# tammypi/flink-siddhi

Measured on AMD Instinct MI355X. Metric: matched-pattern events/sec (whole node) at 1/2/4/8 MI355X + % HBM roofline, higher is better.
Workload: dtype f64+int32+int64

## Files before the change

flink-siddhi_amd/csrc/cf_kernels.hip:

```cpp
#include <hip/hip_runtime.h>

#include "dev_common.h"
#include "kernels.h"
#include "vm.h"

namespace cep {

namespace {

constexpr uint16_t kNoB = 0xffff;
constexpr uint32_t kRolePB = 4;
constexpr int64_t kTolBias = 1ll << 31;
constexpr uint32_t kSkrAlive = 0x8000u;
constexpr int kCfStageBytes = (kCfTile / 8192 * 20 + 36) * 1024;

#ifdef CF_WAVESTAMP
#define CF_STAMP(i) do { } while (0)
#else
#define CF_STAMP(i)                                                                 \
  do {                                                                              \
    if (a.stamps && threadIdx.x == 0 && blockIdx.x < 4096)                          \
      a.stamps[(int64_t)blockIdx.x * 16 + (i)] = __builtin_amdgcn_s_memtime();      \
  } while (0)
#endif

#ifdef CF_WAVESTAMP
#define CF_WSTAMP(slot)                                                             \
  do {                                                                              \
    if (a.stamps && (threadIdx.x & 63) == 0 && blockIdx.x < 4096 && wi == 0 &&     \
        (slot) < 16)                                                                \
      a.stamps[(int64_t)blockIdx.x * 16 + (slot)] = __builtin_amdgcn_s_memtime();  \
  } while (0)
#else
#define CF_WSTAMP(slot) do { } while (0)
#endif

#define CF_COUNT(i, v)                                                                       \
  do {                                                                                       \
    if (a.stamps && (a.ablate & 256))                                                        \
      atomicAdd((unsigned long long*)&a.stamps[4095 * 16 + (i)], (unsigned long long)(v));   \
  } while (0)

template <int E, int Q = kPref>
__device__ __forceinline__ void pick_carried(const uint64_t (&pv)[Q][E], int sa, int sb,
                                             uint32_t role_a, uint64_t (&out)[E]) {
  take_slot<E, Q>(pv, sa, out);
  if (sb != sa) {
#pragma unroll
    for (int q = 0; q < Q; ++q) {
      if (sb == q) {
        asm volatile("");
#pragma unroll
        for (int e = 0; e < E; ++e) out[e] = ((role_a >> e) & 1u) ? out[e] : pv[q][e];
      }
    }
  }
}

__device__ __forceinline__ uint32_t rec_row(uint64_t w0) { return (uint32_t)(w0 >> 32) & 0x1fffu; }
__device__ __forceinline__ uint32_t rec_role(uint64_t w0) { return (uint32_t)(w0 >> 45) & 0x7u; }
__device__ __forceinline__ uint32_t rec_key(uint64_t w0) { return (uint32_t)(w0 >> 48); }

}

#ifndef CF_PART_MINW
#define CF_PART_MINW (kCfPartThreads == 512 ? 4 : 1)
#endif
template <int NW, bool FR, int NP = kPref, bool TOL = false, bool ATL = false>
__global__ __launch_bounds__(kCfPartThreads, CF_PART_MINW) void k_cfpart(CfPartArgs a) {
  constexpr int E = kCfItems, NT = kCfPartThreads, RW = 1 + NW;
  constexpr int kStageBytesT = (FR || TOL || ATL) ? 128 * 1024 : kCfStageBytes;
  constexpr int kStageRecs = kStageBytesT / (8 * RW);
  constexpr uint64_t kHwmBias = 1ull << 63;
  __shared__ uint32_t scratch[NT / 64 + 1];
  __shared__ unsigned long long s_hwm;
  __shared__ unsigned long long s_wmax[NT / 64];
  __shared__ __attribute__((aligned(16))) uint64_t stage[kStageRecs * RW];
  extern __shared__ __attribute__((aligned(16))) uint32_t hist[];
  const int tid = threadIdx.x;
  const int64_t tile = xcd_tile(blockIdx.x, a.ntiles);
  if (TOL && a.gate && *(volatile const uint32_t*)a.gate != a.gate_seq) return;
  const PatternArgs& p = a.pat;
  const bool need_hwm = (ATL && (tile == 0 || tile == a.ntiles - 1)) || (TOL && a.hwm_wr);
  if (need_hwm) {
    if (tid < 64) {
      unsigned long long h = a.hwm_rd ? a.hwm_rd[tid] : 0ull;
#pragma unroll
      for (int o = 32; o > 0; o >>= 1) {
        const unsigned long long y = __shfl_xor(h, o, 64);
        h = y > h ? y : h;
      }
      if (tid == 0) s_hwm = h;
    }
    __syncthreads();
  }
  const int lg = p.buckets_log2;
  const int P = 1 << lg;
  const int NB = P + a.nhot;
  CF_STAMP(0);
  for (int i = tid; i <= NB; i += NT) hist[i] = 0;

  const int64_t ts_base = FR ? (int64_t)a.in_recs[a.rows.row0 * a.in_rec_words + 2] : a.rows.ts[a.rows.row0];
  if (tile == 0 && tid == 0) {
    if (a.pool_cursor) *a.pool_cursor = 0ull;
    a.chunk_base[0] = ts_base;
    a.chunk_base[1] = FR ? (int64_t)a.in_recs[a.rows.row0 * a.in_rec_words + 1] : a.rows.seq0 + a.rows.row0;
  }
  const int lane = tid & 63, wave = tid >> 6;
  const int64_t r0 = tile * kCfTile + (int64_t)wave * 64 * E + lane;
  const int64_t row0 = a.rows.row0 + r0;
  uint32_t valid = 0;
#pragma unroll
  for (int e = 0; e < E; ++e) valid |= (r0 + 64 * e < a.rows.n ? 1u : 0u) << e;
  uint32_t role_a = 0, role_b = 0, role_pb = 0;
  uint64_t tsv[E];
  uint64_t pv[NP][E];
#pragma unroll
  for (int e = 0; e < E; ++e) tsv[e] = 0;
  uint64_t fkey[E], fc0[E], fc1[E];
#pragma unroll
  for (int e = 0; e < E; ++e) fkey[e] = fc0[e] = fc1[e] = 0;
  if (FR && valid) {
    const int rw = a.in_rec_words;
    uint64_t hv[E];
#pragma unroll
    for (int e = 0; e < E; ++e) {
      const bool ok = (valid >> e) & 1u;
      const uint64_t* r = a.in_recs + (row0 + 64 * e) * rw;
      hv[e] = ok ? r[0] : 0ull;
      tsv[e] = ok ? r[2] : 0ull;
      const bool isa = ((hv[e] >> 32) & ROLE_A) != 0;
      fc0[e] = (ok && NW > 0) ? r[3 + (isa ? a.cf.a_log[0] : a.cf.b_log[0])] : 0ull;
      fc1[e] = (ok && NW > 1) ? r[3 + (isa ? a.cf.a_log[1] : a.cf.b_log[1])] : 0ull;
    }
#pragma unroll
    for (int e = 0; e < E; ++e) {
      const uint32_t role = (uint32_t)(hv[e] >> 32) & 0xffu;
      role_a |= ((role & ROLE_A) ? 1u : 0u) << e;
      role_b |= ((role & ROLE_B) && (role & ROLE_G) ? 1u : 0u) << e;
      if (TOL) role_pb |= ((role & ROLE_B) && !(role & ROLE_G) ? 1u : 0u) << e;
      fkey[e] = (uint64_t)(uint32_t)hv[e];
    }
    if (p.within >= 0 && !TOL) {
      const int64_t before = row0 > 0 ? (int64_t)a.in_recs[(row0 - 1) * rw + 2] : batch_prev_ts(a.rows);
      bool bad = false;
#pragma unroll
      for (int e = 0; e < E; ++e) {
        const uint64_t up = __shfl_up(tsv[e], 1, 64);
        const uint64_t last = e > 0 ? __shfl(tsv[e > 0 ? e - 1 : 0], 63, 64) : 0ull;
        const int64_t prev = lane > 0 ? (int64_t)up : (e > 0 ? (int64_t)last : before);
        if ((valid >> e) & 1u) bad |= (int64_t)tsv[e] < prev;
      }
      if (bad) report_descent(a.rows, a.err);
    }
  }
  if (!FR && valid) {
    uint32_t sb[E];
    cf_load_cols<E, NP>(a.rows, a.pref, a.ts_slot, row0, valid, tsv, sb, pv);
    uint32_t is_a = 0, is_b = 0;
#pragma unroll
    for (int e = 0; e < E; ++e) {
      if ((valid >> e) & 1u) {
        is_a |= ((int)sb[e] == p.a_stream ? 1u : 0u) << e;
        is_b |= ((int)sb[e] == p.b_stream ? 1u : 0u) << e;
      }
    }
    if (p.within >= 0 && !TOL) {
      int64_t before;
      if (ATL && r0 == 0) {
        before = (int64_t)(s_hwm ^ kHwmBias);
      } else {
        before = row0 > 0 ? a.rows.ts[row0 - 1] : batch_prev_ts(a.rows);
      }
      bool bad = false;
#pragma unroll
      for (int e = 0; e < E; ++e) {
        const uint64_t up = __shfl_up(tsv[e], 1, 64);
        const uint64_t last = e > 0 ? __shfl(tsv[e > 0 ? e - 1 : 0], 63, 64) : 0ull;
        const int64_t prev = lane > 0 ? (int64_t)up : (e > 0 ? (int64_t)last : before);
        if ((valid >> e) & 1u) bad |= (int64_t)tsv[e] < prev;
      }
      if (bad) {
        if (ATL) *(volatile uint32_t*)a.gate = a.gate_seq;
        else report_descent(a.rows, a.err);
      }
    }
    const uint32_t all = (1u << E) - 1u;
    if (is_a) role_a = is_a & (p.f_prog < 0 ? all : eval_terms_regs<E, NP>(p.f_terms, a.pref.f_slot, a.rows.cols, pv));
    if (is_b) role_b = is_b & (p.g_raw_prog < 0 ? all : eval_terms_regs<E, NP>(p.g_terms, a.pref.g_slot, a.rows.cols, pv));
    if (TOL || ATL) role_pb = is_b & ~role_b;
    if (NW > 0) pick_carried<E, NP>(pv, a.cf.a_slot[0], a.cf.b_slot[0], role_a, fc0);
    if (NW > 1) pick_carried<E, NP>(pv, a.cf.a_slot[1], a.cf.b_slot[1], role_a, fc1);
    if (a.pref.key_slot >= 0) {
#pragma unroll
      for (int e = 0; e < E; ++e) fkey[e] = pv[0][e];
    }
  }
  if (TOL && a.hwm_wr) {
    unsigned long long m = 0ull;
#pragma unroll
    for (int e = 0; e < E; ++e)
      if ((valid >> e) & 1u) m = (tsv[e] ^ kHwmBias) > m ? (tsv[e] ^ kHwmBias) : m;
#pragma unroll
    for (int o = 32; o > 0; o >>= 1) {
      const unsigned long long y = __shfl_xor(m, o, 64);
      m = y > m ? y : m;
    }
    if (lane == 0) s_wmax[wave] = m;
  }
  lds_barrier();
  CF_STAMP(1);
  if (TOL && a.hwm_wr && tid == 0) {
    unsigned long long m = s_hwm;
    for (int w = 0; w < NT / 64; ++w) m = s_wmax[w] > m ? s_wmax[w] : m;
    atomicMax(a.hwm_wr + (tile & 63), m);
  }
  if (ATL && tile == a.ntiles - 1 && tid == 0) {
    const unsigned long long l = (unsigned long long)a.rows.ts[a.rows.row0 + a.rows.n - 1] ^ kHwmBias;
    a.hwm_wr[0] = l > s_hwm ? l : s_hwm;
  }

  uint32_t packed[E];
  uint32_t lkey[E];
#pragma unroll
  for (int e = 0; e < E; ++e) {
    packed[e] = 0xffffffffu;
    lkey[e] = 0;
    const uint32_t role = ((role_a >> e) & 1u) * ROLE_A | ((role_b >> e) & 1u) * ROLE_B |
                          ((TOL || ATL) ? ((role_pb >> e) & 1u) * kRolePB : 0u);
    if (!role) continue;
    int64_t key;
    key = (int64_t)fkey[e];
    const int64_t kfield = shard_key(key, p.key_stride, p.key_offset);
    if (kfield < 0 || kfield >= p.key_capacity) {
      set_err(a.err, ERR_KEY_RANGE);
      continue;
    }
    uint32_t bucket = (uint32_t)(kfield & (P - 1));
    lkey[e] = (uint32_t)(kfield >> lg);
    if (ATL) {
      if (role == kRolePB) bucket += (uint32_t)P;
    } else if (a.nhot) {
      const uint32_t hs = a.hot_id[kfield];
      if (hs != kNotHot) {
        bucket = (uint32_t)P + hs;
        lkey[e] = hs;
      }
    }
    const uint32_t rank = atomicAdd(&hist[bucket], 1u);
    packed[e] = (role << 25) | (bucket << 13) | rank;
  }
  lds_barrier();
  CF_STAMP(2);
  {
    constexpr int MAXPER = kCfMaxBuckets / NT;
    const int per = (NB + NT - 1) / NT;
    uint32_t c[MAXPER];
    uint32_t sum = 0;
#pragma unroll
    for (int i = 0; i < MAXPER; ++i) {
      const int idx = tid * per + i;
      c[i] = (i < per && idx < NB) ? hist[idx] : 0u;
      sum += c[i];
    }
    uint32_t total;
    uint32_t off = bscan<NT>(sum, scratch, &total);
#pragma unroll
    for (int i = 0; i < MAXPER; ++i) {
      const int idx = tid * per + i;
      if (i < per && idx < NB) {
        hist[idx] = off;
        off += c[i];
      }
    }
    if (tid == 0) hist[NB] = total;
  }
  lds_barrier();
  CF_STAMP(3);
  const uint32_t total = hist[NB];
  const uint32_t nreg = ATL ? hist[P] : total;
  const uint32_t words_t = nreg * RW + (total - nreg);
  const bool staged = words_t <= (uint32_t)(kStageRecs * RW);
  uint64_t* trecs = a.recs + tile * (int64_t)kCfTile * RW;
#pragma unroll
  for (int e = 0; e < E; ++e) {
    if (packed[e] == 0xffffffffu) continue;
    const uint32_t b = (packed[e] >> 13) & 0xfffu;
    const uint32_t role = packed[e] >> 25;
    const uint32_t slot = hist[b] + (packed[e] & 0x1fffu);
    const int64_t dts = (int64_t)tsv[e] - ts_base + (TOL ? kTolBias : 0);
    if (dts < 0) {
      if (TOL) set_err(a.err, ERR_TS_SPAN);
      else if (ATL) *(volatile uint32_t*)a.gate = a.gate_seq;
      else report_descent(a.rows, a.err);
    } else if (dts > 0xffffffffll) {
      set_err(a.err, ERR_TS_SPAN);
    }
    const uint64_t w0 = (uint64_t)(uint32_t)dts | ((uint64_t)(wave * 64 * E + 64 * e + lane) << 32) |
                        ((uint64_t)role << 45) | ((uint64_t)lkey[e] << 48);
    const uint64_t c0 = fc0[e], c1 = fc1[e];
    if (ATL && b >= (uint32_t)P) {
      const uint32_t wd = nreg * RW + (slot - nreg);
      if (staged) stage[wd] = w0;
      else trecs[wd] = w0;
      continue;
    }
    if (staged) {
      stage[slot * RW] = w0;
      if (NW > 0) stage[slot * RW + 1] = c0;
      if (NW > 1) stage[slot * RW + 2] = c1;
    } else {
      uint64_t* g = trecs + (int64_t)slot * RW;
      g[0] = w0;
      if (NW > 0) g[1] = c0;
      if (NW > 1) g[2] = c1;
    }
  }
  for (int i = tid; i <= NB; i += NT) a.tile_off[(int64_t)i * a.ntiles + tile] = (uint16_t)hist[i];
  if (staged) {
    lds_barrier();
    CF_STAMP(4);
    const int64_t words = (int64_t)words_t;
    for (int64_t w = 2 * tid; w < words; w += 2 * NT) {
      if (w + 1 < words) *(uint4*)(trecs + w) = *(const uint4*)(stage + w);
      else trecs[w] = stage[w];
    }
  }
  CF_STAMP(5);
}

#if !defined(CF_UNIT) || CF_UNIT == 1
constexpr int kCfRouteStage = 112 * 1024;
constexpr int kRouteSmallWorld = 8;
__global__ __launch_bounds__(kCfPartThreads, 1) void k_cfroute(CfRouteArgs ca) {
  constexpr int E = kCfItems, NT = kCfPartThreads, NWV = NT / 64;
  const RouteArgs& a = ca.r;
  const PatternArgs& p = a.pat;
  __shared__ uint32_t wcnt[NWV][kMaxWorld];
  __shared__ uint32_t obase[kMaxWorld + 1];
  __shared__ __attribute__((aligned(16))) uint64_t stage[kCfRouteStage / 8];
  const int tid = threadIdx.x, lane = tid & 63, wave = tid >> 6;
  const int world = a.world, wrw = a.wrw;
  const int64_t tile = blockIdx.x;
  for (int i = tid; i < NWV * kMaxWorld; i += NT) wcnt[i / kMaxWorld][i % kMaxWorld] = 0;

  const int64_t r0 = tile * kCfTile + (int64_t)wave * 64 * E + lane;
  const int64_t row0 = a.rows.row0 + r0;
  uint32_t valid = 0;
#pragma unroll
  for (int e = 0; e < E; ++e) valid |= (r0 + 64 * e < a.rows.n ? 1u : 0u) << e;
  uint64_t tsv[E], pv[kPref][E];
#pragma unroll
  for (int e = 0; e < E; ++e) tsv[e] = 0;
  uint32_t is_a = 0, role_a = 0, role_b = 0, role_g = 0;
  uint64_t fkey[E], fc0[E], fc1[E];
#pragma unroll
  for (int e = 0; e < E; ++e) fkey[e] = fc0[e] = fc1[e] = 0;
  if (valid) {
    uint32_t sb[E];
    cf_load_cols<E>(a.rows, ca.pref, ca.ts_slot, row0, valid, tsv, sb, pv);
    uint32_t is_b = 0;
#pragma unroll
    for (int e = 0; e < E; ++e) {
      if ((valid >> e) & 1u) {
        is_a |= ((int)sb[e] == p.a_stream ? 1u : 0u) << e;
        is_b |= ((int)sb[e] == p.b_stream ? 1u : 0u) << e;
      }
    }
    const uint32_t all = (1u << E) - 1u;
    if (is_a) role_a = is_a & (p.f_prog < 0 ? all : eval_terms_regs<E>(p.f_terms, ca.pref.f_slot, a.rows.cols, pv));
    if (is_b) {
      if (p.g_walk_prog >= 0) {
        role_b = is_b;
      } else {
        role_g = is_b & (p.g_raw_prog < 0 ? all : eval_terms_regs<E>(p.g_terms, ca.pref.g_slot, a.rows.cols, pv));
        role_b = p.tolerant ? is_b : role_g;
      }
    }
    if (p.nrec_a > 0 || p.nrec_b > 0)
      pick_carried<E>(pv, p.nrec_a > 0 ? ca.pref.reca_slot[0] : -1, p.nrec_b > 0 ? ca.pref.recb_slot[0] : -1,
                      is_a, fc0);
    if (p.nrec_a > 1 || p.nrec_b > 1)
      pick_carried<E>(pv, p.nrec_a > 1 ? ca.pref.reca_slot[1] : -1, p.nrec_b > 1 ? ca.pref.recb_slot[1] : -1,
                      is_a, fc1);
    if (ca.pref.key_slot >= 0) {
#pragma unroll
      for (int e = 0; e < E; ++e) fkey[e] = pv[0][e];
    }
  }
  __syncthreads();

  const uint64_t lt = (lane == 0) ? 0ull : (~0ull >> (64 - lane));
  int dest[E];
  uint32_t wr[E];
  uint32_t pre[kRouteSmallWorld];
#pragma unroll
// ... 1178 lines not shown
```

flink-siddhi_amd/csrc/dev_common.h:

```cpp
#pragma once
#include <hip/hip_runtime.h>

#include "kernels.h"
#include "vm.h"

namespace cep {
namespace {

__device__ __forceinline__ void set_err(unsigned int* err, unsigned int bit) {
  if (err) atomicOr(err, bit);
}

__device__ __forceinline__ int64_t batch_prev_ts(const RowsArgs& r) {
  int64_t p = r.prev_ts;
  if (r.prev_ts_dev) {
    const int64_t d = *r.prev_ts_dev;
    p = d > p ? d : p;
  }
  return p;
}

__device__ __forceinline__ void report_descent(const RowsArgs&, unsigned int* err) {
  set_err(err, ERR_ORDER);
}
// ... 57 lines not shown
  lds_barrier();
  const uint32_t r = scratch[wave] + x - v;
  *total = scratch[NWV];
  if (kTail) lds_barrier();
  return r;
}

__device__ __forceinline__ int64_t shard_key(int64_t key, int32_t stride, int32_t offset) {
  if (stride == 1) return (key < 0 || offset != 0) ? -1 : key;
  if (key < 0 || key > 0xffffffffll) return -1;
  const uint32_t k = (uint32_t)key, q = k / (uint32_t)stride;
  return (k - q * (uint32_t)stride) == (uint32_t)offset ? (int64_t)q : -1;
}

template <int E>
__device__ __forceinline__ void load_raw(const void* p, int w, int64_t row, uint4 (&r)[E / 2]) {
  const char* b = (const char*)p + row * w;
  const int nl = w == 8 ? E / 2 : (w == 4 ? (E / 4 > 0 ? E / 4 : 1) : 1);
#pragma unroll
  for (int i = 0; i < E / 2; ++i) r[i] = gload4(b + 16 * (i < nl ? i : nl - 1));
}

template <int E>
__device__ __forceinline__ void decode(const uint4 (&r)[E / 2], int type, uint64_t (&v)[E]) {
  uint32_t x[2 * E];
#pragma unroll
  for (int i = 0; i < E / 2; ++i) {
    x[4 * i] = r[i].x;
    x[4 * i + 1] = r[i].y;
    x[4 * i + 2] = r[i].z;
    x[4 * i + 3] = r[i].w;
  }
  if (type == T_LONG || type == T_DOUBLE) {
#pragma unroll
    for (int e = 0; e < E; ++e) v[e] = ((uint64_t)x[2 * e + 1] << 32) | x[2 * e];
  } else if (type == T_BOOL) {
#pragma unroll
    for (int e = 0; e < E; ++e) v[e] = ((x[e >> 2] >> (8 * (e & 3))) & 0xffu) ? 1u : 0u;
  } else if (type == T_FLOAT) {
#pragma unroll
    for (int e = 0; e < E; ++e) v[e] = (uint64_t)x[e];
  } else {
#pragma unroll
    for (int e = 0; e < E; ++e) v[e] = from_i32((int32_t)x[e]);
  }
}

template <int N, int Q = kPref>
__device__ __forceinline__ uint64_t pick(const uint64_t (&v)[Q][N], int slot, int e) {
  uint64_t x = 0;
#pragma unroll
  for (int q = 0; q < Q; ++q) x |= v[q][e] & (0ull - (uint64_t)(slot == q));
  return x;
}

template <int N, int Q = kPref>
__device__ __forceinline__ void take_slot(const uint64_t (&v)[Q][N], int slot, uint64_t (&out)[N]) {
#pragma unroll
  for (int e = 0; e < N; ++e) out[e] = 0;
#pragma unroll
  for (int q = 0; q < Q; ++q) {
    if (slot == q) {
      asm volatile("");
#pragma unroll
      for (int e = 0; e < N; ++e) out[e] = v[q][e];
    }
  }
}

template <int N, int Q = kPref>
__device__ __forceinline__ uint32_t eval_terms_regs(const TermList& tl, const int32_t* slot,
                                                    const ColSet& cols,
                                                    const uint64_t (&vals)[Q][N]) {
  uint32_t acc = tl.any ? 0u : ((N >= 32) ? 0xffffffffu : ((1u << N) - 1u));
#pragma unroll
  for (int i = 0; i < kMaxTerms; ++i) {
    if (i >= tl.n) break;
    const Term& t = tl.t[i];
    uint64_t v[N];
    take_slot<N, Q>(vals, slot[i], v);
    int ty = (t.coltype == T_BOOL || t.coltype == T_STRING) ? T_INT : t.coltype;
    uint32_t nullm = 0;
    if (t.aop) {
      convert_run<N>(v, ty, t.atype);
      arith_run<N>(v, t.aop, t.atype, t.aconst, &nullm);
      ty = t.atype;
    }
    convert_run<N>(v, ty, t.ctype);
    const uint32_t bits = compare_run<N>(v, t.cop, t.ctype, t.cconst) & ~nullm;
    acc = tl.any ? (acc | bits) : (acc & bits);
  }
  return acc;
}

__device__ __forceinline__ const uint64_t* granule(const void* base, int64_t row, int w) {
  const char* b = (const char*)base;
  const int64_t mis = (int64_t)((uintptr_t)b & 7u);
  const int64_t off = row * w + mis;
  return (const uint64_t*)(b - mis + (w == 8 ? off : (off & ~(int64_t)7)));
}
__device__ __forceinline__ uint64_t from_granule(uint64_t g, const void* base, int64_t row, int type) {
  const int w = type_width(type);
  if (w == 8) return g;
  const uint32_t sh = (uint32_t)((row * w + (int64_t)((uintptr_t)base & 7u)) & 7) * 8u;
  const uint32_t x = (uint32_t)(g >> sh);
  if (w == 1) return (x & 0xffu) ? 1ull : 0ull;
  return type == T_FLOAT ? (uint64_t)x : from_i32((int32_t)x);
}

template <int E, int Q = kPref>
__device__ __forceinline__ void cf_load_cols(const RowsArgs& rows, const PrefPlan& pref, int ts_slot,
                                             int64_t row0, uint32_t valid, uint64_t (&tsv)[E],
                                             uint32_t (&sb)[E], uint64_t (&pv)[Q][E]) {
#pragma unroll
  for (int e = 0; e < E; ++e) {
    const bool ok = (valid >> e) & 1u;
    tsv[e] = ok ? (uint64_t)rows.ts[row0 + 64 * e] : 0ull;
    sb[e] = (ok && rows.stream) ? (uint32_t)rows.stream[row0 + 64 * e] : (uint32_t)rows.input;
  }
#pragma unroll
  for (int q = 0; q < Q; ++q) {
    const int c = pref.col[q];
    const int ty = rows.cols.t[c];
    if (q < pref.n && q != ts_slot) {
      const void* base = rows.cols.p[c];
      if (ty == T_LONG || ty == T_DOUBLE) {
#pragma unroll
        for (int e = 0; e < E; ++e)
          pv[q][e] = ((valid >> e) & 1u) ? ((const uint64_t*)base)[row0 + 64 * e] : 0ull;
      } else if (ty == T_BOOL) {
#pragma unroll
        for (int e = 0; e < E; ++e)
          pv[q][e] = ((valid >> e) & 1u) ? (((const uint8_t*)base)[row0 + 64 * e] ? 1ull : 0ull) : 0ull;
      } else {
#pragma unroll
        for (int e = 0; e < E; ++e) {
          const uint32_t v = ((valid >> e) & 1u) ? ((const uint32_t*)base)[row0 + 64 * e] : 0u;
          pv[q][e] = ty == T_FLOAT ? (uint64_t)v : from_i32((int32_t)v);
        }
      }
    } else {
#pragma unroll
      for (int e = 0; e < E; ++e) pv[q][e] = 0;
    }
  }
#pragma unroll
  for (int q = 0; q < Q; ++q)
    if (q == ts_slot) {
#pragma unroll
      for (int e = 0; e < E; ++e) pv[q][e] = tsv[e];
    }
}

__device__ __forceinline__ uint32_t wave_incl_scan(uint32_t x) {
  x += (uint32_t)__builtin_amdgcn_update_dpp(0, (int)x, 0x111, 0xf, 0xf, false);
  x += (uint32_t)__builtin_amdgcn_update_dpp(0, (int)x, 0x112, 0xf, 0xf, false);
  x += (uint32_t)__builtin_amdgcn_update_dpp(0, (int)x, 0x114, 0xf, 0xf, false);
  x += (uint32_t)__builtin_amdgcn_update_dpp(0, (int)x, 0x118, 0xf, 0xf, false);
  x += (uint32_t)__builtin_amdgcn_update_dpp(0, (int)x, 0x142, 0xa, 0xf, false);
  x += (uint32_t)__builtin_amdgcn_update_dpp(0, (int)x, 0x143, 0xc, 0xf, false);
  return x;
}

__device__ __forceinline__ int xcd_tile(int bid, int n) {
  if (n < 8 || (n & 7)) return bid;
  return (bid & 7) * (n >> 3) + (bid >> 3);
}

__device__ __forceinline__ int xcd_bucket(int bid, int nb) {
  if (nb < 8 || (nb & 7)) return bid;
  return (bid & 7) * (nb >> 3) + (bid >> 3);
}

}
}
```

flink-siddhi_amd/csrc/engine.cpp:

```cpp
#include <hip/hip_runtime.h>

#include <algorithm>
#include <cstdio>
#include <cstdlib>
#include <cstring>
#include <memory>
#include <numeric>
#include <string>
#include <unordered_map>
#include <vector>

#include "../../include/cep.h"
#include "frontend.h"
#include "kernels.h"

using namespace cep;

namespace {

struct DevBuf {
  void* p = nullptr;
  size_t bytes = 0;
};

// ... 1092 lines not shown
      uint64_t tc = 1;
      while (tc < 2 * (uint64_t)kc) tc <<= 1;
      rt.sparse = true;
      rt.table_cap = tc;
      if (!dev_ensure(&rt.tkey, tc * 8, a->stream, false) || !dev_ensure(&rt.tval, tc * 4, a->stream, false) ||
          !dev_ensure(&rt.krev, (size_t)kc * 8, a->stream, false) || !dev_ensure(&rt.kcount, 64, a->stream, false))
        return fail(a, CEP_E_DEVICE, "out of device memory (key map)");
      hipMemset(rt.tkey.p, 0, tc * 8);
      hipMemset(rt.tval.p, 0xff, tc * 4);
      hipMemset(rt.kcount.p, 0, 4);
      hipMemset((char*)rt.kcount.p + 4, 0xff, 4);
    }
    rt.order_sensitive = p.within >= 0 && !agg && !(q.nfa && q.sequence);
    a->pats.push_back(rt);
  }
  {
    const int64_t none = INT64_MIN;
    if (!dev_ensure(&a->last_ts_dev, 64, a->stream, false) ||
        hipMemcpy(a->last_ts_dev.p, &none, 8, hipMemcpyHostToDevice) != hipSuccess)
      return fail(a, CEP_E_DEVICE, "out of device memory");
  }
  if (std::getenv("CEP_STAMPS") && !dev_ensure(&a->stamps, (size_t)2 * 4096 * 16 * 8, a->stream, false))
    return fail(a, CEP_E_DEVICE, "out of device memory (stamps)");
  hipStreamSynchronize(a->stream);
  return CEP_OK;
}

const StreamSchema* find_schema(cep_app* a, const char* id) {
  if (!id) return nullptr;
  int i = a->app.input_index(id);
  if (i >= 0) return &a->app.inputs[i];
  i = a->app.output_index(id);
  if (i >= 0) return &a->app.outputs[i];
  return nullptr;
}

int fill_attrs(const StreamSchema* s, cep_attr* out, int cap, int* n) {
  if (n) *n = (int)s->attrs.size();
  for (int i = 0; i < (int)s->attrs.size() && i < cap; ++i) {
    std::snprintf(out[i].name, sizeof(out[i].name), "%s", s->attrs[i].name.c_str());
    out[i].type = s->attrs[i].type;
  }
  return CEP_OK;
}

int run_filter(cep_app* a, const Query& q, const RowsArgs& rows) {
  OutStream& o = a->outs[a->app.output_index(q.out_stream)];
  o.bound += rows.n;
  int rc = ensure_out_cap(a, o, o.bound);
  if (rc) return rc;
  constexpr int64_t kTile = kFilterThreads * kFilterItems;
  const int64_t ntiles = (rows.n + kTile - 1) / kTile;
  if (ntiles == 0) return CEP_OK;
  const int64_t fcr = filterc_rows_per_tile();
  const int64_t nflags = std::max<int64_t>(ntiles, (rows.n + fcr - 1) / fcr);
  if (!dev_ensure(&a->tile_state, (size_t)nflags * 8, a->stream, false))
    return fail(a, CEP_E_DEVICE, "out of device memory (tile state)");
  hipMemsetAsync(a->tile_state.p, 0, (size_t)nflags * 8, a->stream);
  hipMemsetAsync(a->ticket.p, 0, 16, a->stream);
  FilterArgs fa{};
  fa.rows = rows;
  fa.vm = {(const Ins*)a->code.p, (const uint64_t*)a->konst.p};
  fa.in_stream = q.in_stream;
  fa.filter_prog = q.filter.off;
  fa.filter_terms = q.filter_terms;
  fa.out = out_args(o, q);
  fa.tile_state = (unsigned long long*)a->tile_state.p;
  fa.ticket = (unsigned int*)a->ticket.p;
  fa.err = (unsigned int*)a->err.p;
  bool vm = q.filter.off >= 0 && q.filter_terms.n < 0;
  for (auto& it : q.select) vm |= it.src < SRC_REC || it.src >= SRC_TS;
  static const bool no_fc = std::getenv("CEP_NO_FILTERC") != nullptr;
  bool fc = !vm && !no_fc && (rows.row0 & 1) == 0;
  if (fc) {
    fa.npref = 0;
    for (int i = 0; fc && i < std::max(0, q.filter_terms.n); ++i) {
      const int c = q.filter_terms.t[i].col;
      int slot = -1;
      for (int k = 0; k < fa.npref; ++k)
        if (fa.pcol[k] == c) slot = k;
      if (slot < 0) {
        if (fa.npref == 3) {
          fc = false;
          break;
        }
        slot = fa.npref;
        fa.pcol[fa.npref++] = c;
      }
      fa.fslot[i] = slot;
    }
    if (fa.npref == 0) fa.pcol[fa.npref++] = 0;
    auto al = [&](const void* ptr, int w) {
      return (((uintptr_t)ptr + (uintptr_t)(rows.row0 * w)) & (uintptr_t)(2 * w - 1)) == 0;
    };
    for (int k = 0; fc && k < fa.npref; ++k)
      fc = al(rows.cols.p[fa.pcol[k]], type_width(rows.cols.t[fa.pcol[k]]));
    if (fc && rows.stream) fc = al(rows.stream, 1);
  }
  LaunchTimer t(a, CEP_K_FILTER);
  if (fc) {
    const int64_t tr = filterc_rows_per_tile();
    const int64_t nt = (rows.n + tr - 1) / tr;
    launch_filterc(fa, nt, a->stream);
  } else {
    launch_filter(fa, ntiles, vm, a->stream);
  }
  return CEP_OK;
}

bool pref_aligned(const PrefPlan& pf, const RowsArgs& rows) {
  auto al = [&](const void* ptr, int w) {
    const uintptr_t need = w == 1 ? 7u : 15u;
    return (((uintptr_t)ptr + (uintptr_t)(rows.row0 * w)) & need) == 0;
  };
  bool ok = al(rows.ts, 8) && (!rows.stream || al(rows.stream, 1));
  for (int i = 0; i < pf.n; ++i) {
    const int c = pf.col[i];
    ok = ok && al(rows.cols.p[c], type_width(rows.cols.t[c]));
  }
  return ok;
}

bool cf_plan(const PatternRT& rt, const RowsArgs& rows, CfPlan* cf, bool from_records = false) {
  const PatternArgs& p = rt.pa;
  std::memset(cf, 0, sizeof(*cf));
  int a_phys[kMaxCaps], b_phys[kMaxCaps];
  int na = 0, nb = 0;
  auto alias = [&](int col) {
    return !from_records && rows.cols.p[col] == (const void*)rows.ts && rows.cols.t[col] == T_LONG;
  };
  for (int c = 0; c < p.nrec_a; ++c) {
    a_phys[c] = alias(p.rec_a[c]) ? -1 : na;
    if (a_phys[c] >= 0) {
      cf->a_log[na] = c;
      cf->a_slot[na++] = rt.pref.reca_slot[c];
    }
  }
  for (int c = 0; c < p.nrec_b; ++c) {
    b_phys[c] = alias(p.rec_b[c]) ? -1 : nb;
    if (b_phys[c] >= 0) {
      cf->b_log[nb] = c;
      cf->b_slot[nb++] = rt.pref.recb_slot[c];
    }
  }
  cf->nw = std::max(na, nb);
  if (cf->nw > 2) return false;
  for (int w = na; w < 2; ++w) cf->a_slot[w] = 0;
  for (int w = nb; w < 2; ++w) cf->b_slot[w] = 0;
  for (int i = 0; i < kMaxCaps; ++i) cf->cap_phys[i] = i < p.ncap ? a_phys[p.cap_from_rec[i]] : 0;
  for (int c = 0; c < kMaxCaps; ++c) cf->bcol_phys[c] = c < p.nrec_b ? b_phys[c] : 0;
  return true;
}

int run_pattern_cf(cep_app* a, PatternRT& rt, const Query& q, OutStream& o,
                   const RowsArgs& rows_all, const CfPlan& cf,
                   const uint64_t* in_recs = nullptr, int in_rec_words = 0, bool tol = false) {
  const int P = 1 << rt.pa.buckets_log2;
  const bool hot_ok = rt.hot;
  static const bool overlap = std::getenv("CEP_OVERLAP") != nullptr;
  hipStream_t side = overlap ? a->side : a->stream;
  if (overlap) {
    hipEventRecord(a->in_ready, a->stream);
    hipStreamWaitEvent(a->side, a->in_ready, 0);
  }
  constexpr int64_t kHotProbeRows = 1 << 20;
  for (int64_t r0 = 0, step = 0; r0 < rows_all.n; r0 += step) {
    const int b = rt.cur;
    rt.cur ^= 1;
    const bool probe = hot_ok && !rt.hot_on && !rt.hot_probed;
    step = std::min<int64_t>(probe ? std::min<int64_t>(kHotProbeRows, rt.cf_chunk) : rt.cf_chunk, rows_all.n - r0);
    RowsArgs rows = rows_all;
    rows.row0 = rows_all.row0 + r0;
    rows.n = step;
    if (r0 > 0) rows.prev_ts = INT64_MIN;
    const int64_t ntiles = (rows.n + kCfTile - 1) / kCfTile;
    CfPartArgs pa{};
    pa.rows = rows;
    pa.pref = rt.pref;
    pa.ts_slot = -1;
    pa.in_recs = in_recs;
    pa.in_rec_words = in_rec_words;
    for (int i = 0; i < rt.pref.n && !in_recs; ++i)
      if (rows.cols.p[rt.pref.col[i]] == (const void*)rows.ts && rows.cols.t[rt.pref.col[i]] == T_LONG)
        pa.ts_slot = i;
    pa.pat = rt.pa;
    pa.pat.tolerant = tol ? 1 : 0;
    pa.cf = cf;
    pa.chunk_base = (int64_t*)rt.chunk_base[b].p;
    pa.recs = (uint64_t*)rt.cf_recs[b].p;
    pa.tile_off = (uint16_t*)rt.cf_toff[b].p;
    pa.ntiles = (int32_t)ntiles;
    pa.err = (unsigned int*)a->err.p;
    pa.pool_cursor = overlap ? nullptr : (unsigned long long*)rt.pool_cur.p;
    if (overlap) hipMemsetAsync(rt.pool_cur.p, 0, 8, a->stream);
    if (a->stamps.p) pa.stamps = (uint64_t*)a->stamps.p + 4096 * 16;
    const bool hot = hot_ok;
    if (hot && !rt.hot_on && *(volatile uint32_t*)rt.hot_active_host.p > 0) {
      const int rw = 1 + cf.nw;
      const int64_t cc = rt.cf_chunk, ntmax = cc / kCfTile;
      rt.hot_blocks = (int)((cc + kHotBlock - 1) / kHotBlock);
      const bool ok = dev_ensure(&rt.hot_gbase, (kCfHotMax + 1) * 4, a->stream, false) &&
                      dev_ensure(&rt.hoff, (size_t)kCfHotMax * ntmax * 4, a->stream, false) &&
                      dev_ensure(&rt.harr, (size_t)cc * rw * 8, a->stream, false) &&
                      dev_ensure(&rt.hrow, (size_t)cc * 4, a->stream, false) &&
                      dev_ensure(&rt.hnb, (size_t)cc * 4, a->stream, false) &&
                      dev_ensure(&rt.bsum, (size_t)rt.hot_blocks * 16, a->stream, false) &&
                      dev_ensure(&rt.bcnt, (size_t)rt.hot_blocks * 4, a->stream, false) &&
                      dev_ensure(&rt.boff, (size_t)rt.hot_blocks * 4, a->stream, false) &&
                      dev_ensure(&rt.hcm, kCfHotMax * 3 * 4, a->stream, false) &&
                      dev_ensure(&rt.hobase, 64, a->stream, false) &&
                      dev_ensure(&rt.htmn, (size_t)cc * 4, a->stream, false) &&
                      dev_ensure(&rt.htmx, (size_t)cc * 4, a->stream, false) &&
                      dev_ensure(&rt.hflag, (size_t)cc, a->stream, false) &&
                      dev_ensure(&rt.btol, (size_t)rt.hot_blocks * 12, a->stream, false);
      if (!ok) return fail(a, CEP_E_DEVICE, "out of device memory (hot-key arenas)");
      rt.hot_on = true;
    }
    const bool divert = hot && rt.hot_on;
    pa.hot_id = divert ? (const uint16_t*)rt.hot_id.p : nullptr;
    pa.nhot = divert ? kCfHotMax : 0;
    static const bool no_atol = std::getenv("CEP_NO_ATOL") != nullptr;
    const bool atol = tol && !in_recs && !divert && rt.atol_ok && rt.hwm.p && !no_atol &&
                      (2 << rt.pa.buckets_log2) <= kCfMaxBuckets && q.a_stream != q.b_stream;
    uint32_t gseq = 0;
    if (tol && rt.hwm.p) {
      const int par = (int)(rt.tol_chunks++ & 1);
      pa.hwm_rd = (const unsigned long long*)rt.hwm.p + (par ^ 1) * 64;
      pa.hwm_wr = (unsigned long long*)rt.hwm.p + par * 64;
    }
    if (atol) {
      if (++rt.atol_seq == 0) ++rt.atol_seq;
      gseq = rt.atol_seq;
      pa.gate = (uint32_t*)rt.atol_gate.p;
      pa.gate_seq = gseq;
    }
    if (overlap && rt.used[b]) hipStreamWaitEvent(side, rt.walk_done[b], 0);
    if (overlap && hot && rt.used[b ^ 1]) hipStreamWaitEvent(side, rt.walk_done[b ^ 1], 0);
    if (atol) {
      CfPartArgs aa = pa;
      aa.atol = 1;
      aa.pat.tolerant = 0;
      aa.nhot = P;
      aa.hot_id = nullptr;
      LaunchTimer t(a, CEP_K_CF_PARTITION, side);
      launch_cf_partition(aa, ntiles, side);
    }
    {
      LaunchTimer t(a, atol ? CEP_K_OTHER : CEP_K_CF_PARTITION, side);
      launch_cf_partition(pa, ntiles, side);
    }
    if (overlap) {
      hipEventRecord(rt.part_done[b], side);
      hipStreamWaitEvent(a->stream, rt.part_done[b], 0);
    }
    CfWalkArgs wa{};
    wa.pat = pa.pat;
    wa.cf = cf;
    wa.recs = pa.recs;
    wa.tile_off = pa.tile_off;
    wa.ntiles = (int32_t)ntiles;
    wa.chunk_base = (const int64_t*)rt.chunk_base[b].p;
    wa.khdr = (uint32_t*)rt.khdr.p;
    wa.kslot = (uint64_t*)rt.kslot.p;
    wa.kstride = rt.kstride;
    wa.kext = (uint64_t*)rt.kext.p;
    wa.pool_rd = (const uint64_t*)rt.pool[rt.pool_side].p;
    wa.pool_wr = (uint64_t*)rt.pool[rt.pool_side ^ 1].p;
    wa.pool_cursor = (unsigned long long*)rt.pool_cur.p;
    wa.pool_cap = (uint64_t)rt.pool_cap;
    wa.key_rev = rt.sparse ? (const uint64_t*)rt.krev.p : nullptr;
    wa.out = out_args(o, q);
    wa.err = pa.err;
    HotArgs ha{};
    if (hot) {
      ha.pat = pa.pat;
      ha.cf = cf;
      ha.recs = pa.recs;
      ha.tile_off = pa.tile_off;
      ha.ntiles = (int32_t)ntiles;
      ha.chunk_base = (const int64_t*)rt.chunk_base[b].p;
      ha.hot_id = (uint16_t*)rt.hot_id.p;
      ha.hot_key = (int32_t*)rt.hot_key.p;
      ha.hot_m = (uint32_t*)rt.hot_m.p;
      ha.hot_gbase = (uint32_t*)rt.hot_gbase.p;
      ha.hoff = (uint32_t*)rt.hoff.p;
      ha.cand = (uint64_t*)rt.cand.p;
      ha.ncand = (uint32_t*)rt.ncand.p;
      ha.cand_cap = kCfHotMax * 4;
      ha.thresh = rt.hot_thresh;
      ha.harr = (uint64_t*)rt.harr.p;
      ha.hrow = (uint32_t*)rt.hrow.p;
      ha.hnb = (uint32_t*)rt.hnb.p;
      ha.bsum = (uint32_t*)rt.bsum.p;
      ha.bcnt = (uint32_t*)rt.bcnt.p;
      ha.boff = (uint32_t*)rt.boff.p;
      ha.hcm = (uint32_t*)rt.hcm.p;
      ha.obase = (unsigned long long*)rt.hobase.p;
      ha.htmn = (uint32_t*)rt.htmn.p;
      ha.htmx = (uint32_t*)rt.htmx.p;
      ha.hflag = (uint8_t*)rt.hflag.p;
      ha.btol = (uint32_t*)rt.btol.p;
      ha.max_blocks = rt.hot_blocks;
      ha.khdr = wa.khdr;
      ha.kslot = wa.kslot;
      ha.kstride = wa.kstride;
      ha.kext = wa.kext;
      ha.pool_rd = wa.pool_rd;
      ha.pool_wr = wa.pool_wr;
      ha.pool_cursor = wa.pool_cursor;
      ha.pool_cap = wa.pool_cap;
      ha.key_rev = wa.key_rev;
      ha.out = wa.out;
      ha.active = (uint32_t*)rt.hot_active.p;
      ha.in_seq = in_recs ? in_recs + rows.row0 * in_rec_words + 1 : nullptr;
      ha.in_rec_words = in_rec_words;
      static const int hot_ablate = std::getenv("CEP_HOT_ABLATE") ? std::atoi(std::getenv("CEP_HOT_ABLATE")) : 0;
      ha.ablate = hot_ablate;
      ha.err = pa.err;
      wa.hot_cand = ha.cand;
      wa.hot_ncand = ha.ncand;
      wa.hot_thresh = rt.hot_thresh;
      wa.hot_id = divert ? ha.hot_id : nullptr;
    }
    static const bool hot_serial = std::getenv("CEP_HOT_SERIAL") != nullptr;
    hipStream_t hs = hot_serial ? a->stream : a->side;
    if (divert) {
      if (!hot_serial) {
        hipEventRecord(rt.hot_fork, a->stream);
        hipStreamWaitEvent(hs, rt.hot_fork, 0);
      }
      {
        LaunchTimer t(a, CEP_K_HOT, hs);
        launch_hot_match(ha, hs);
      }
      if (!hot_serial) hipEventRecord(rt.hot_join, hs);
    }
    wa.in_seq = in_recs ? in_recs + rows.row0 * in_rec_words + 1 : nullptr;
    wa.in_rec_words = in_rec_words;
    static const int ablate = std::getenv("CEP_ABLATE") ? std::atoi(std::getenv("CEP_ABLATE")) : 0;
    wa.ablate = ablate;
    if (a->stamps.p) {
      wa.stamps = (uint64_t*)a->stamps.p;
      hipMemsetAsync(wa.stamps, 0, (size_t)4096 * 16 * 8, a->stream);
    }
    if (atol) {
// ... 2029 lines not shown
```

flink-siddhi_amd/csrc/kernels.h:

```cpp
#pragma once
#include <hip/hip_runtime.h>

#include <cstdint>

#include "plan.h"

namespace cep {

struct ColSet {
  const void* p[kMaxCols];
  int32_t t[kMaxCols];
  int32_t n;
};

struct RowsArgs {
  ColSet cols;
  const int64_t* ts;
  const uint8_t* stream;
  int32_t input;
  int64_t row0;
  int64_t n;
  int64_t seq0;
  int64_t prev_ts;
  const int64_t* seq;
// ... 90 lines not shown
  int32_t st_stream[kMaxStates];
  int32_t st_min[kMaxStates], st_max[kMaxStates];
  int32_t st_raw[kMaxStates];
  int32_t st_walk[kMaxStates];
  int32_t st_tail_opt[kMaxStates];
  int32_t key_col_s[8];
  int32_t cap_state[kMaxCaps], cap_index[kMaxCaps], cap_word[kMaxCaps];
  uint64_t cap_null[kMaxCaps];
};

constexpr int kPfRec = 2;
struct PrefPlan {
  int32_t n = -1;
  int32_t col[kPref];
  int32_t f_slot[kMaxTerms], g_slot[kMaxTerms];
  int32_t key_slot = -1;
  int32_t reca_slot[8], recb_slot[8];
};

struct PartArgs {
  RowsArgs rows;
  PrefPlan pref;
  VmArgs vm;
  PatternArgs pat;
  int32_t from_records;
  const uint64_t* in_recs;
  int32_t in_rec_words;
  int64_t* chunk_base;
  int32_t tile_rows;
  uint64_t* recs;
  uint16_t* tile_off;
  uint64_t* stamps;
  unsigned int* err;
};

constexpr int kMaxWorld = 64;

struct RowRouteArgs {
  RowsArgs rows;
  int32_t world;
  int32_t wrw;
  int32_t tile_rows;
  int64_t seq0;
  int32_t key_col_s[8];
  uint64_t* arena;
  uint32_t* tcount;
  unsigned int* err;
  int64_t seg_cap;
  uint64_t* spill;
  int64_t spill_cap;
  int64_t* spill_counts;
};

constexpr uint32_t kRowNullStream = 31;

struct RowUnpackArgs {
  const uint64_t* recs;
  int64_t n;
  int32_t wrw;
  int32_t ncols;
  void* col[kMaxCols];
  int32_t type[kMaxCols];
  int64_t* ts;
  uint8_t* stream;
  int64_t* seq;
};
struct RouteArgs {
  RowsArgs rows;
  VmArgs vm;
  PatternArgs pat;
  int32_t world;
  int32_t wrw;
  int32_t tile_rows;
  int64_t seq0;
  uint64_t* arena;
  uint32_t* tcount;
  unsigned int* err;
  int64_t seg_cap;
  int32_t row_mode;
  uint64_t* spill;
  int64_t spill_cap;
  int64_t* spill_counts;
};

struct WalkArgs {
  VmArgs vm;
  PatternArgs pat;
  const uint64_t* recs;
  const uint16_t* tile_off;
  int32_t ntiles;
  int32_t tile_rows;
  const int64_t* chunk_base;
  uint32_t* khdr;
  uint64_t* kslot;
  int64_t kstride;
  uint64_t* stamps;
  OutArgs out;
  unsigned int* err;
  uint64_t* kext;
  const uint64_t* pool_rd;
  uint64_t* pool_wr;
  unsigned long long* pool_cursor;
  uint64_t pool_cap;
};

#ifndef CF_TILE_ROWS
#define CF_TILE_ROWS 8192
#endif
constexpr int kCfItems = 8;
constexpr int kCfPartThreads = CF_TILE_ROWS / kCfItems;
constexpr int kCfTile = CF_TILE_ROWS;
constexpr int kCfWalkThreads = 512;
constexpr int kCfWindow = 2048;
constexpr int kCfMaxKeys = 512;
constexpr int kCfMaxTiles = (32 << 20) / kCfTile;
constexpr int kCfMaxBuckets = 4096;
constexpr int kCfMaxCaps = 2;
constexpr int kCfMaxOut = 8;

struct CfPlan {
  int32_t nw;
  int32_t a_slot[2], b_slot[2];
  int32_t a_log[2], b_log[2];
  int32_t cap_phys[kMaxCaps];
  int32_t bcol_phys[kMaxCaps];
};

constexpr int kCfHotMax = 1024;
constexpr int kHotBlock = 2048;
constexpr uint16_t kNotHot = 0xffff;

struct CfPartArgs {
  RowsArgs rows;
  const uint16_t* hot_id;
  int32_t nhot;
  PrefPlan pref;
  int32_t ts_slot;
  const uint64_t* in_recs;
  int32_t in_rec_words;
  PatternArgs pat;
  CfPlan cf;
  int64_t* chunk_base;
  uint64_t* recs;
  uint16_t* tile_off;
  int32_t ntiles;
  uint64_t* stamps;
  unsigned int* err;
  int32_t atol;
  uint32_t* gate;
  uint32_t gate_seq;
  const unsigned long long* hwm_rd;
  unsigned long long* hwm_wr;
  unsigned long long* pool_cursor;
};

struct CfWalkArgs {
  PatternArgs pat;
  CfPlan cf;
  const uint64_t* recs;
  const uint16_t* tile_off;
  int32_t ntiles;
  const int64_t* chunk_base;
  uint32_t* khdr;
  uint64_t* kslot;
  int64_t kstride;
  uint64_t* kext;
  const uint64_t* pool_rd;
  uint64_t* pool_wr;
  unsigned long long* pool_cursor;
  uint64_t pool_cap;
  const uint64_t* key_rev;
  const uint16_t* hot_id;
  uint64_t* hot_cand;
  uint32_t* hot_ncand;
  uint32_t hot_thresh;
  OutArgs out;
  const uint64_t* in_seq;
  int32_t in_rec_words;
  uint64_t* stamps;
  int32_t ablate;
  unsigned int* err;
  int32_t atol;
  const uint32_t* gate;
  uint32_t gate_seq;
};

struct HotArgs {
  PatternArgs pat;
  CfPlan cf;
  const uint64_t* recs;
  const uint16_t* tile_off;
  int32_t ntiles;
  const int64_t* chunk_base;
  uint16_t* hot_id;
  int32_t* hot_key;
  uint32_t* hot_m;
  uint32_t* hot_gbase;
  uint32_t* hoff;
  uint64_t* cand;
  uint32_t* ncand;
  uint32_t cand_cap;
  uint32_t thresh;
  uint64_t* harr;
  uint32_t* hrow;
  uint32_t* hnb;
  uint32_t* bsum;
  uint32_t* bcnt;
  uint32_t* boff;
  uint32_t* hcm;
  uint32_t* htmn;
  uint32_t* htmx;
  uint8_t* hflag;
  uint32_t* btol;
  unsigned long long* obase;
  int32_t max_blocks;
  uint32_t* khdr;
  uint64_t* kslot;
  int64_t kstride;
  uint64_t* kext;
  const uint64_t* pool_rd;
  uint64_t* pool_wr;
  unsigned long long* pool_cursor;
  uint64_t pool_cap;
  const uint64_t* key_rev;
  OutArgs out;
  uint32_t* active;
  const uint64_t* in_seq;
  int32_t in_rec_words;
  int32_t ablate;
  unsigned int* err;
};

struct CfRouteArgs {
  RouteArgs r;
  PrefPlan pref;
  int32_t ts_slot;
};

struct KeyMapArgs {
  const void* key;
  int32_t key_is_long;
  const uint8_t* stream;
  int32_t input, a_stream, b_stream;
  int64_t row0, n;
  unsigned long long* tkey;
  uint32_t* tval;
  uint64_t table_cap;
  uint64_t* rev;
  unsigned int* count;
  unsigned int* minus_one;
  uint32_t cap;
  int32_t* out;
  unsigned int* err;
};

struct RouteKeyArgs {
  const void* col;
  int32_t type;
  int64_t n;
  const int32_t* str_hash;
  int32_t nstr;
  int32_t nchan;
  int64_t seq0;
  int64_t* keys;
  int32_t* chan;
};

constexpr int kMqMaxQ = 64;
constexpr int kMqMaxCond = 47;
constexpr int kMqTrueBit = 47;
constexpr int kMqMaxCarry = 4;
constexpr int kMqMaxPhys = 4;
constexpr int kMqMaxCaps = 4;
constexpr int kMqMaxSel = 8;
constexpr int kMqMaxAggs = 4;
constexpr int kMqTile = 16384;
constexpr int kMqPartThreads = 1024;
constexpr int kMqWalkThreads = 1024;
constexpr int kMqWindow = 4096;
constexpr int kMqMaxTiles = (16 << 20) / kMqTile;
constexpr int kMqMaxKpb = 1024;
constexpr int kMqMaxBuckets = 8192;
constexpr int mq_window(int nc) { return nc <= 0 ? 4096 : nc == 1 ? 3072 : nc <= 3 ? 2048 : 1536; }
constexpr int kMqStgWords = 320;
enum : int32_t { MQ_SEQ = 0, MQ_AGG = 1 };
enum : int32_t { MQ_SRC_KEY = 14, MQ_SRC_TS = 15 };

struct MqCond {
  TermList tl;
  int32_t slot[kMaxTerms];
};

struct MqQuery {
  int32_t kind;
  int32_t nwords;
  int64_t st_off;
  int32_t nstates, every;
  int64_t within;
  uint32_t stream_mask;
  uint32_t st_stream;
  uint64_t st_bit;
  uint64_t st_min, st_max;
  uint32_t tail_opt;
  int32_t ncap;
  int32_t cap_state[kMqMaxCaps], cap_last[kMqMaxCaps], cap_src[kMqMaxCaps];
  int32_t in_stream, filter_bit, nagg;
  int32_t agg_fn[kMqMaxAggs], agg_arg_type[kMqMaxAggs], agg_out_type[kMqMaxAggs], agg_src[kMqMaxAggs];
// ... 122 lines not shown
```

Measured before the change: 48.73 billion.

## Stagger early partition blocks, add full-tile column loader, batch hot-id lookups, drop unused ts slot

Adds a timed start delay for the first 256 partition blocks so they do not all hit HBM at once, enabled by default with an env-overridable value. Full tiles now use a loader with no per-element validity masks that also fetches the previous timestamp. Hot-id gathers are hoisted into one unrolled loop so the loads can be in flight together. On the host, the timestamp column is removed from the prefetch plan when no filter, key or window slot uses it, which saves one column load. The stagger adds deliberate idle time to some blocks and could cost throughput if the contention it targets is small.

```diff
diff --git a/flink-siddhi_amd/csrc/cf_kernels.hip b/flink-siddhi_amd/csrc/cf_kernels.hip
--- a/flink-siddhi_amd/csrc/cf_kernels.hip
+++ b/flink-siddhi_amd/csrc/cf_kernels.hip
@@ -80,6 +80,11 @@
   const int tid = threadIdx.x;
   const int64_t tile = xcd_tile(blockIdx.x, a.ntiles);
   if (TOL && a.gate && *(volatile const uint32_t*)a.gate != a.gate_seq) return;
+  if (a.stagger > 0 && blockIdx.x < kCfStaggerBlocks) {
+    const uint64_t t0 = __builtin_amdgcn_s_memtime();
+    const uint64_t d = (uint64_t)((blockIdx.x >> 3) & 31u) * (uint64_t)a.stagger;
+    while (__builtin_amdgcn_s_memtime() - t0 < d) __builtin_amdgcn_s_sleep(8);
+  }
   const PatternArgs& p = a.pat;
   const bool need_hwm = (ATL && (tile == 0 || tile == a.ntiles - 1)) || (TOL && a.hwm_wr);
   if (need_hwm) {
@@ -154,9 +159,12 @@
       if (bad) report_descent(a.rows, a.err);
     }
   }
+  const bool full = !FR && (tile + 1) * (int64_t)kCfTile <= a.rows.n;
   if (!FR && valid) {
     uint32_t sb[E];
-    cf_load_cols<E, NP>(a.rows, a.pref, a.ts_slot, row0, valid, tsv, sb, pv);
+    int64_t before_full = 0;
+    if (full) cf_load_cols_full<E, NP>(a.rows, a.pref, a.ts_slot, row0, tsv, sb, pv, &before_full);
+    else cf_load_cols<E, NP>(a.rows, a.pref, a.ts_slot, row0, valid, tsv, sb, pv);
     uint32_t is_a = 0, is_b = 0;
 #pragma unroll
     for (int e = 0; e < E; ++e) {
@@ -169,6 +177,8 @@
       int64_t before;
       if (ATL && r0 == 0) {
         before = (int64_t)(s_hwm ^ kHwmBias);
+      } else if (full) {
+        before = row0 > 0 ? before_full : batch_prev_ts(a.rows);
       } else {
         before = row0 > 0 ? a.rows.ts[row0 - 1] : batch_prev_ts(a.rows);
       }
@@ -222,6 +232,17 @@
 
   uint32_t packed[E];
   uint32_t lkey[E];
+  uint32_t hsv[E];
+#pragma unroll
+  for (int e = 0; e < E; ++e) hsv[e] = kNotHot;
+  if (!ATL && a.nhot) {
+#pragma unroll
+    for (int e = 0; e < E; ++e) {
+      const bool role = (((role_a | role_b | (TOL ? role_pb : 0u)) >> e) & 1u) != 0;
+      const int64_t kfield = shard_key((int64_t)fkey[e], p.key_stride, p.key_offset);
+      hsv[e] = a.hot_id[(role && kfield >= 0 && kfield < p.key_capacity) ? kfield : 0];
+    }
+  }
 #pragma unroll
   for (int e = 0; e < E; ++e) {
     packed[e] = 0xffffffffu;
@@ -241,7 +262,7 @@
     if (ATL) {
       if (role == kRolePB) bucket += (uint32_t)P;
     } else if (a.nhot) {
-      const uint32_t hs = a.hot_id[kfield];
+      const uint32_t hs = hsv[e];
       if (hs != kNotHot) {
         bucket = (uint32_t)P + hs;
         lkey[e] = hs;
diff --git a/flink-siddhi_amd/csrc/dev_common.h b/flink-siddhi_amd/csrc/dev_common.h
--- a/flink-siddhi_amd/csrc/dev_common.h
+++ b/flink-siddhi_amd/csrc/dev_common.h
@@ -233,6 +233,68 @@
     }
 }
 
+template <int E, int Q = kPref>
+__device__ __forceinline__ void cf_load_cols_full(const RowsArgs& rows, const PrefPlan& pref, int ts_slot,
+                                                  int64_t row0, uint64_t (&tsv)[E], uint32_t (&sb)[E],
+                                                  uint64_t (&pv)[Q][E], int64_t* before) {
+  const int64_t* tp = rows.ts + row0;
+  *before = rows.ts[row0 > 0 ? row0 - 1 : 0];
+#pragma unroll
+  for (int e = 0; e < E; ++e) tsv[e] = (uint64_t)tp[64 * e];
+  const uint8_t* sp = rows.stream ? rows.stream + row0 : (const uint8_t*)tp;
+  uint32_t sraw[E];
+#pragma unroll
+  for (int e = 0; e < E; ++e) sraw[e] = (uint32_t)sp[64 * e];
+  uint32_t lo[Q][E], hi[Q][E];
+#pragma unroll
+  for (int q = 0; q < Q; ++q) {
+    const int c = pref.col[q];
+    const int ty = rows.cols.t[c];
+    const void* base = rows.cols.p[c];
+    if (q < pref.n && q != ts_slot && (ty == T_LONG || ty == T_DOUBLE)) {
+      const uint64_t* b = (const uint64_t*)base + row0;
+#pragma unroll
+      for (int e = 0; e < E; ++e) {
+        const uint64_t x = b[64 * e];
+        lo[q][e] = (uint32_t)x;
+        hi[q][e] = (uint32_t)(x >> 32);
+      }
+    } else if (q < pref.n && q != ts_slot && ty == T_BOOL) {
+      const uint8_t* b = (const uint8_t*)base + row0;
+#pragma unroll
+      for (int e = 0; e < E; ++e) {
+        lo[q][e] = (uint32_t)b[64 * e];
+        hi[q][e] = 0;
+      }
+    } else if (q < pref.n && q != ts_slot) {
+      const uint32_t* b = (const uint32_t*)base + row0;
+#pragma unroll
+      for (int e = 0; e < E; ++e) {
+        lo[q][e] = b[64 * e];
+        hi[q][e] = 0;
+      }
+    } else {
+#pragma unroll
+      for (int e = 0; e < E; ++e) lo[q][e] = hi[q][e] = 0;
+    }
+  }
+#pragma unroll
+  for (int e = 0; e < E; ++e) sb[e] = rows.stream ? sraw[e] : (uint32_t)rows.input;
+#pragma unroll
+  for (int q = 0; q < Q; ++q) {
+    const int ty = rows.cols.t[pref.col[q]];
+    const bool wide = ty == T_LONG || ty == T_DOUBLE;
+    const bool sext = !wide && ty != T_BOOL && ty != T_FLOAT;
+    const bool isb = ty == T_BOOL;
+#pragma unroll
+    for (int e = 0; e < E; ++e) {
+      const uint32_t l = isb ? (lo[q][e] ? 1u : 0u) : lo[q][e];
+      const uint32_t h = sext ? (uint32_t)((int32_t)lo[q][e] >> 31) : hi[q][e];
+      pv[q][e] = q == ts_slot ? tsv[e] : (((uint64_t)h << 32) | l);
+    }
+  }
+}
+
 __device__ __forceinline__ uint32_t wave_incl_scan(uint32_t x) {
   x += (uint32_t)__builtin_amdgcn_update_dpp(0, (int)x, 0x111, 0xf, 0xf, false);
   x += (uint32_t)__builtin_amdgcn_update_dpp(0, (int)x, 0x112, 0xf, 0xf, false);
diff --git a/flink-siddhi_amd/csrc/engine.cpp b/flink-siddhi_amd/csrc/engine.cpp
--- a/flink-siddhi_amd/csrc/engine.cpp
+++ b/flink-siddhi_amd/csrc/engine.cpp
@@ -1268,6 +1268,34 @@
   return true;
 }
 
+void cf_drop_ts_slot(CfPartArgs* pa) {
+  const int ts = pa->ts_slot;
+  PrefPlan& pf = pa->pref;
+  if (ts < 0 || pa->in_recs || pf.n < 2 || pf.key_slot == ts) return;
+  const PatternArgs& p = pa->pat;
+  const int nf = p.f_prog >= 0 ? p.f_terms.n : 0, ng = p.g_raw_prog >= 0 ? p.g_terms.n : 0;
+  for (int i = 0; i < nf; ++i)
+    if (pf.f_slot[i] == ts) return;
+  for (int i = 0; i < ng; ++i)
+    if (pf.g_slot[i] == ts) return;
+  for (int w = 0; w < pa->cf.nw; ++w)
+    if (pa->cf.a_slot[w] == ts || pa->cf.b_slot[w] == ts) return;
+  auto down = [&](int32_t& s) {
+    if (s > ts) --s;
+  };
+  for (int i = ts; i + 1 < pf.n; ++i) pf.col[i] = pf.col[i + 1];
+  --pf.n;
+  for (int i = pf.n; i < kPref; ++i) pf.col[i] = pf.col[0];
+  for (int i = 0; i < nf; ++i) down(pf.f_slot[i]);
+  for (int i = 0; i < ng; ++i) down(pf.g_slot[i]);
+  for (int w = 0; w < 2; ++w) {
+    down(pa->cf.a_slot[w]);
+    down(pa->cf.b_slot[w]);
+  }
+  down(pf.key_slot);
+  pa->ts_slot = -1;
+}
+
 int run_pattern_cf(cep_app* a, PatternRT& rt, const Query& q, OutStream& o,
                    const RowsArgs& rows_all, const CfPlan& cf,
                    const uint64_t* in_recs = nullptr, int in_rec_words = 0, bool tol = false) {
@@ -1302,11 +1330,14 @@
     pa.pat = rt.pa;
     pa.pat.tolerant = tol ? 1 : 0;
     pa.cf = cf;
+    cf_drop_ts_slot(&pa);
     pa.chunk_base = (int64_t*)rt.chunk_base[b].p;
     pa.recs = (uint64_t*)rt.cf_recs[b].p;
     pa.tile_off = (uint16_t*)rt.cf_toff[b].p;
     pa.ntiles = (int32_t)ntiles;
     pa.err = (unsigned int*)a->err.p;
+    static const int stagger = std::getenv("CEP_CF_STAGGER") ? std::atoi(std::getenv("CEP_CF_STAGGER")) : 1280;
+    pa.stagger = ntiles >= 4 * kCfStaggerBlocks ? stagger : 0;
     pa.pool_cursor = overlap ? nullptr : (unsigned long long*)rt.pool_cur.p;
     if (overlap) hipMemsetAsync(rt.pool_cur.p, 0, 8, a->stream);
     if (a->stamps.p) pa.stamps = (uint64_t*)a->stamps.p + 4096 * 16;
diff --git a/flink-siddhi_amd/csrc/kernels.h b/flink-siddhi_amd/csrc/kernels.h
--- a/flink-siddhi_amd/csrc/kernels.h
+++ b/flink-siddhi_amd/csrc/kernels.h
@@ -266,7 +266,9 @@
   const unsigned long long* hwm_rd;
   unsigned long long* hwm_wr;
   unsigned long long* pool_cursor;
-};
+  int32_t stagger;
+};
+constexpr int kCfStaggerBlocks = 256;
 
 struct CfWalkArgs {
   PatternArgs pat;
```

Result: faster. 50.85 billion, median of 6 (+4.4%).
